# hpc-fci-mackenzie/cfrk

Measured on AMD Instinct MI355X. Metric: k-mers/sec, higher is better.
Workload: dtype u64; 1 GPU; 100000000 synthetic 150 bp reads, k=31, canonical, genome 100000000 (BASELINE.json configs[2]); reads=100000000, read_len=150, k=31, parallelism=read-shard x1

## Files before the change

### cfrk_amd/csrc/msp.hip

```cpp
#include "msp.h"
#include "table.h"
#include "msp_dev.h"

#include <algorithm>
#include <cmath>
#include <new>
#include <type_traits>
#include <vector>

namespace {
#include "msp_runs.h"

constexpr int P1_THREADS = 512;

constexpr int P2_THREADS = 512, P2_PER = 8;
constexpr int P2_GROUP = 4;

constexpr int P3_THREADS = 1024;
constexpr int TS_LOG = 12, TS = 1 << TS_LOG;

__device__ __noinline__ void spill_record(uint4 rec, int k, bool canon, TableView t, uint32_t weight = 1u) {
  t.stats[ST_SPILLED] = 1;
  dev_count_event(&t.stats[ST_AUX0]);
  const int nk = (int)(rec.w & 63u) + 1;
  const uint64_t hi = ((uint64_t)rec.x << 32) | rec.y;
  const uint64_t lo = (uint64_t)rec.z << 32;
  for (int j = 0; j < nk; ++j) {
    const uint64_t x = j ? ((hi << (2 * j)) | (lo >> (64 - 2 * j))) : hi;
    uint64_t key = x >> (64 - 2 * k);
    if (canon) {
      const uint64_t rc = dev_revcomp64(key, k);
      key = rc < key ? rc : key;
    }
    table_add1(t, key, weight);
  }
}

constexpr int P1_OWN = 61;
constexpr int P1_WAVES = P1_THREADS / 64;

__host__ __device__ __forceinline__ uint32_t l1_reg(uint32_t bin, uint32_t xg) { return xg * (uint32_t)B1 + bin; }
template <bool SUB>
__device__ __forceinline__ uint32_t bin_of(uint32_t w) { return SUB ? ((w >> 16) & (uint32_t)(B1 - 1)) : (w >> 16); }

template <bool EX>
__device__ __forceinline__ void l1_put(const MspView &v, uint32_t reg, uint32_t dst, uint4 rec, int k, bool canon,
                                       const TableView &t) {
  const bool exact1 = EX && v.exact1;
  const uint64_t cap = exact1 ? (uint64_t)v.rcap[reg] : v.cap1;
  const uint64_t at = exact1 ? v.rbase[reg] : (uint64_t)reg * v.cap1;
  if (dst < cap) {
    v.rec1[at + dst] = rec;
  } else if (exact1) {
    spill_record(rec, k, canon, t);
  } else if (*(volatile uint64_t *)&v.stats[ST_L1OVF] == 0) {
    const unsigned long long o = atomicAdd((unsigned long long *)&v.stats[ST_OVFN1], 1ull);
    if (o < v.ovf1_cap) v.ovf1[o] = rec;
    else v.stats[ST_L1OVF] = 1;
  }
}

constexpr int SUB_BITS = 5;
#define P1_MARK(text) asm volatile("; " text)
template <int P1B_TR, bool SUB = false>
struct P1Lds {
  static constexpr int STAGE = 4096 + 3 * 512 + P1B_TR * 128 + (SUB ? 2048 : 0);
  static constexpr int ARENA = P1_WAVES * STAGE;
  static constexpr int BYTES = ARENA + 2 * B1 * 4 + 32;
};

template <int W, int P1B_TR, bool EX, bool SUB>
__device__ __forceinline__ void p1_tile(uint4 *pool, const int8_t *__restrict__ data, int64_t nN, int k, int m, int canon,
                                        int64_t tile, uint32_t subreg, const MspView &v, const TableView &t) {
  constexpr int NH = 32 + W - 1;
  constexpr int P1B_STAGE = P1Lds<P1B_TR, SUB>::STAGE;
  constexpr int P1B_TAIL = B1 * 10;
  constexpr int P1B_RCAP = (P1_WAVES * P1B_STAGE - P1B_TAIL) / 16;
  uint4 *const arena = pool;
  uint32_t *const hist = reinterpret_cast<uint32_t *>(reinterpret_cast<uint8_t *>(pool) + P1Lds<P1B_TR, SUB>::ARENA);
  uint32_t *const loff = hist + B1;
  uint32_t *const wtot = loff + B1;
  uint32_t *const nrec_p = wtot + 4;
  uint32_t *const gbase = hist;
  unsigned long long *const dabs = reinterpret_cast<unsigned long long *>(reinterpret_cast<uint8_t *>(arena) + P1B_RCAP * 16);
  uint16_t *const plim = reinterpret_cast<uint16_t *>(dabs + B1);
  static_assert((P1_WAVES * P1B_STAGE - P1B_TAIL) % 16 == 0, "the table starts on a record boundary");

  const int nkmax = min(48 - k + 1, 32);
  const int tid = threadIdx.x, lane = tid & 63, wave = tid >> 6;
  uint8_t *const stage = reinterpret_cast<uint8_t *>(arena) + wave * P1B_STAGE;
  uint32_t *const s_str = reinterpret_cast<uint32_t *>(stage);
  uint4 *const s_EW = reinterpret_cast<uint4 *>(stage + 512);
  uint16_t *const s_leaf = reinterpret_cast<uint16_t *>(stage + 1536);
  uint16_t *const s_dsc = reinterpret_cast<uint16_t *>(stage + 4096 + 1536);
  uint8_t *const s_sub = stage + 4096 + 1536 + P1B_TR * 128;
  if (tid < B1) hist[tid] = 0;
  lds_barrier();

  P1_MARK("P1_PHASE_A");
  const int64_t wave_g = tile * P1_WAVES + wave;
  const int64_t chunk = wave_g * P1_OWN + lane - 1;
  const int64_t off = chunk * 32;
  uint32_t b0 = 0, b1 = 0, bad = 0xFFFFFFFFu;
  if (chunk >= 0) {
    if (off + 32 > nN) P1_MARK("P1_COLD byte-wise tail chunk");
    dev_load_chunk32(data, off, nN, b0, b1, bad);
  }
  const uint32_t n0 = dev_lane_next(b0), n1 = dev_lane_next(b1);
  const uint32_t nbad = dev_lane_next(bad), nnbad = dev_lane_next(dev_lane_next(bad));
  const uint64_t hi = ((uint64_t)b0 << 32) | b1;
  const uint64_t mid = ((uint64_t)n0 << 32) | n1;
  uint64_t Yh = ((uint64_t)bad << 32) | nbad, Yl = (uint64_t)nnbad << 32;
  {
    int w = 1;
#pragma unroll
    for (int st = 0; st < 5; ++st) {
      if (2 * w <= k) {
        Yh |= (Yh << w) | (Yl >> (64 - w));
        Yl |= Yl << w;
        w *= 2;
      }
    }
    if (k > w) {
      Yh |= (Yh << (k - w)) | (Yl >> (64 - (k - w)));
      Yl |= Yl << (k - w);
    }
  }
  const uint64_t Vx = ~Yh;
  const uint32_t V = (uint32_t)(Vx >> 32);
  const uint32_t prevV = dev_lane_prev(V) & 1u;

  uint32_t H[NH];
  const uint64_t Cx = msp_minimizers<W>(hi, mid, chunk, m, H);
  const uint64_t E = Cx | ~Vx | (1ull << (63 - NH));
  const uint32_t Vprev = (V >> 1) | (prevV << 31);
  uint32_t S = V & ((uint32_t)(Cx >> 32) | ~Vprev);
  const bool owner = lane >= 1 && lane <= P1_OWN && off < nN;
  if (!owner) S = 0;

  P1_MARK("P1_PHASE_B1");
  {
    const LeafPack LP = leaf_pack(H);
    uint4 *lp = reinterpret_cast<uint4 *>(s_leaf + lane * 32);
    lp[0] = make_uint4(LP.w[0], LP.w[1], LP.w[2], LP.w[3]);
    lp[1] = make_uint4(LP.w[4], LP.w[5], LP.w[6], LP.w[7]);
    lp[2] = make_uint4(LP.w[8], LP.w[9], LP.w[10], LP.w[11]);
    lp[3] = make_uint4(LP.w[12], LP.w[13], LP.w[14], LP.w[15]);
    reinterpret_cast<uint2 *>(s_str)[lane] = make_uint2(b0, b1);
    s_EW[lane] = make_uint4((uint32_t)E, (uint32_t)(E >> 32), ((uint32_t)Vx >> 1) | (V << 31), Vprev);
    if (SUB) {
      uint32_t sw[8];
#pragma unroll
      for (int i = 0; i < 8; ++i) {
        uint32_t x = 0;
#pragma unroll
        for (int j = 3; j >= 0; --j) {
          const uint32_t h = H[4 * i + j];
          x = (x << 8) | (((h >> 24) & 15u) << 1) | ((h >> 7) & 1u);
        }
        sw[i] = x;
      }
      uint4 *sp = reinterpret_cast<uint4 *>(s_sub + lane * 32);
      sp[0] = make_uint4(sw[0], sw[1], sw[2], sw[3]);
      sp[1] = make_uint4(sw[4], sw[5], sw[6], sw[7]);
    }
  }
  if (v.dbg & CFRK_ABL_P1_NO_EMIT) {
    if (S == 0x12345678u && (uint32_t)E == 0x9ABCDEFu) v.stats[ST_AUX0] = 1;
    return;
  }
  uint32_t cnt_w;
  uint32_t S2 = 0;
  const uint32_t wcap = (v.dbg & CFRK_DEBUG_SMALL_WAVE_CAP) ? 64u : (uint32_t)(P1B_TR * 64);
  {
    const uint32_t mine = (uint32_t)__popc(S);
    const uint32_t incl = dev_wave_scan_incl(mine);
    cnt_w = (uint32_t)__builtin_amdgcn_readlane((int)incl, 63);
    uint32_t widx = incl - mine;
    const uint32_t tag = (uint32_t)lane << 5;
    if (incl <= wcap) {
      uint16_t *dp = s_dsc + widx - 1;
      while (S) {
        const int a = __clz(S);
        S &= ~(0x80000000u >> a);
        *++dp = (uint16_t)(tag | (uint32_t)a);
      }
    } else {
      P1_MARK("P1_COLD wave over capacity");
      while (S) {
        const int a = __clz(S);
        const uint32_t bit = 0x80000000u >> a;
        S &= ~bit;
        if (widx < wcap) s_dsc[widx] = (uint16_t)(tag | (uint32_t)a);
        else S2 |= bit;
        ++widx;
      }
    }
  }
  lds_wave_sync();

  const uint32_t nkm1 = (uint32_t)(nkmax - 1);
  const int zc = 2 * (48 - k);
  auto build = [&](uint32_t d) {
    const uint4 ew = s_EW[d >> 5];
    const uint32_t leaf = s_leaf[d];
    const uint32_t idx0 = (d - 1u) >> 4, sh = 0u - 2u * d;
    const uint32_t D0 = s_str[idx0], D1 = s_str[idx0 + 1], D2 = s_str[idx0 + 2], D3 = s_str[idx0 + 3];
    const uint32_t a = d & 31u, na = ~d;
    const uint32_t e32 = __builtin_amdgcn_alignbit(ew.y, ew.x, na);
    const uint32_t nm1 = min((uint32_t)__clz(e32), nkm1);
    const uint32_t lf = (ew.w >> (na & 31u)) & 1u;
    const uint64_t Ws = ((uint64_t)ew.w << 32) | ew.z;
    const uint32_t rf = (uint32_t)((Ws << (a + nm1 + 2u)) >> 63);
    uint4 rec;
    rec.x = __builtin_amdgcn_alignbit(D0, D1, sh);
    const int z = zc - 2 * (int)nm1;
    uint64_t r12 = ((uint64_t)__builtin_amdgcn_alignbit(D1, D2, sh) << 32) | __builtin_amdgcn_alignbit(D2, D3, sh);
    r12 = (W < 8 && z >= 64) ? 0ull : (r12 & (~0ull << z));
    rec.y = (uint32_t)(r12 >> 32);
    rec.z = (uint32_t)r12;
    rec.w = (leaf << 8) | (rf << 7) | (lf << 6) | nm1;
    if (SUB) rec.w |= (uint32_t)s_sub[d] << 24;
    return rec;
  };

  while (S2) {
    P1_MARK("P1_COLD direct append");
    const int a = __clz(S2);
    S2 &= ~(0x80000000u >> a);
    const uint4 rec = build(((uint32_t)lane << 5) | (uint32_t)a);
    if (((rec.w >> 8) & v.sel_mask) != v.sel_val) continue;
    const uint32_t reg = l1_reg(bin_of<SUB>(rec.w), subreg);
    const uint32_t dst = atomicAdd(&v.cnt1[reg], 1u);
    l1_put<EX>(v, reg, dst, rec, k, canon != 0, t);
  }

  P1_MARK("P1_PHASE_B2");
  uint4 rc[P1B_TR];
  uint32_t rk[P1B_TR];
  cnt_w = min(cnt_w, wcap);
  auto emit = [&](auto sel) {
    if (decltype(sel)::value) P1_MARK("P1_COLD multi-pass selection");
#pragma unroll
    for (int tr = 0; tr < P1B_TR; ++tr) {
      rk[tr] = 0xFFFFFFFFu;
      const uint32_t i = (uint32_t)(tr * 64 + lane);
      if (i < cnt_w) {
        rc[tr] = build(s_dsc[i]);
        if (!decltype(sel)::value || ((rc[tr].w >> 8) & v.sel_mask) == v.sel_val)
          rk[tr] = atomicAdd(&hist[bin_of<SUB>(rc[tr].w)], 1u);
      }
    }
  };
  if (v.sel_mask == 0 && v.sel_val == 0) emit(std::false_type{});
  else emit(std::true_type{});
  lds_barrier();

  P1_MARK("P1_PHASE_C");
  uint32_t my_base = 0;
  if (tid < B1) {
    const uint32_t c = hist[tid];
    if (c) my_base = atomicAdd(&v.cnt1[l1_reg(tid, subreg)], c);
  }
  block_scan<B1, true>(hist, loff, wtot);
  if (tid == B1 - 1) *nrec_p = loff[tid] + hist[tid];
#pragma unroll
  for (int tr = 0; tr < P1B_TR; ++tr) {
    if (rk[tr] != 0xFFFFFFFFu) {
      const uint32_t pos = loff[bin_of<SUB>(rc[tr].w)] + rk[tr];
      if (pos < (uint32_t)P1B_RCAP) arena[pos] = rc[tr];
    }
  }
  if (tid < B1) {
    gbase[tid] = my_base;
    const uint32_t reg = l1_reg(tid, subreg);
    const bool exact1 = EX && v.exact1;
    const uint64_t cap = exact1 ? (uint64_t)v.rcap[reg] : v.cap1;
    const uint64_t at = exact1 ? v.rbase[reg] : (uint64_t)reg * v.cap1;
    const uint32_t lo = loff[tid];
    dabs[tid] = at + my_base - lo;
    const uint64_t room = cap > (uint64_t)my_base ? cap - my_base : 0;
    plim[tid] = (uint16_t)min((uint64_t)lo + room, (uint64_t)0xFFFFu);
    static_assert(P1B_RCAP <= 0xFFFF, "arena positions fit 16 bits");
  }
  lds_barrier();

  P1_MARK("P1_PHASE_D");
  const uint32_t nrec_s = *nrec_p;
  const uint32_t nrec = min(nrec_s, (uint32_t)P1B_RCAP);
  for (uint32_t p = tid; p < nrec; p += P1_THREADS) {
    const uint4 rec = arena[p];
    const uint32_t b = bin_of<SUB>(rec.w);
    if (p < (uint32_t)plim[b]) {
      v.rec1[dabs[b] + p] = rec;
    } else {
      P1_MARK("P1_COLD region full");
      l1_put<EX>(v, l1_reg(b, subreg), gbase[b] + (p - loff[b]), rec, k, canon != 0, t);
    }
  }
  if (nrec_s > (uint32_t)P1B_RCAP) {
    P1_MARK("P1_COLD arena overflow");
#pragma unroll
    for (int tr = 0; tr < P1B_TR; ++tr) {
      if (rk[tr] != 0xFFFFFFFFu) {
        const uint32_t b = bin_of<SUB>(rc[tr].w);
        if (loff[b] + rk[tr] >= (uint32_t)P1B_RCAP)
          l1_put<EX>(v, l1_reg(b, subreg), gbase[b] + rk[tr], rc[tr], k, canon != 0, t);
      }
    }
  }
}

template <int W, int P1B_TR, bool SUB>
__global__ __launch_bounds__(P1_THREADS, ((P1B_TR <= 6 && !SUB) ? 6 : 4)) void msp_p1b_kernel(const int8_t *__restrict__ data,
                                                             int64_t nN, int k, int m, int canon,
                                                             int64_t tile0, MspView v, TableView t) {
  __shared__ uint4 pool[P1Lds<P1B_TR, SUB>::BYTES / 16];
  const int64_t tile = tile0 + blockIdx.x;
  p1_tile<W, P1B_TR, true, SUB>(pool, data, nN, k, m, canon, tile, (uint32_t)tile & (v.nxg - 1), v, t);
}

constexpr int NCLS = 2;
constexpr int NSUB = NCLS * B2;
__device__ __forceinline__ uint32_t sub_of(uint32_t w) { return (((w >> 8) & (B2 - 1)) << 1) | ((((w >> 6) & 3u) == 3u) ? 1u : 0u); }

template <int PER>
struct P2Lds {
  static constexpr int TILE = P2_THREADS * PER;
  static constexpr int DABS = TILE * 16;
  static constexpr int HIST = DABS + NSUB * 8;
  static constexpr int LOFF = HIST + NSUB * 4;
  static constexpr int PLIM = LOFF + NSUB * 4;
  static constexpr int WTOT = PLIM + NSUB * 2;
  static constexpr int RPRE = WTOT + (P2_THREADS / 64) * 4;
  static constexpr int GPRE = RPRE + (NXG + 1) * 4;
  static constexpr int BYTES = (GPRE + (B1 / NXCD + 1) * 4 + 15) / 16 * 16;
};

template <int PER, bool EX, bool PF, int NGRP>
__device__ __forceinline__ void p2_item(uint4 *pool, uint32_t b1, uint32_t grp, int k, int canon, const MspView &v, const TableView &t) {
  constexpr int TILE = P2_THREADS * PER;
  static_assert(TILE <= 0xFFFF, "tile positions fit 16 bits");
  uint4 *const sorted = pool;
  uint8_t *const pb = reinterpret_cast<uint8_t *>(pool);
  unsigned long long *const dabs = reinterpret_cast<unsigned long long *>(pb + P2Lds<PER>::DABS);
  uint32_t *const hist = reinterpret_cast<uint32_t *>(pb + P2Lds<PER>::HIST);
  uint32_t *const loff = reinterpret_cast<uint32_t *>(pb + P2Lds<PER>::LOFF);
  uint16_t *const plim = reinterpret_cast<uint16_t *>(pb + P2Lds<PER>::PLIM);
  uint32_t *const wtot = reinterpret_cast<uint32_t *>(pb + P2Lds<PER>::WTOT);
  uint32_t *const rpre = reinterpret_cast<uint32_t *>(pb + P2Lds<PER>::RPRE);
  static_assert(NSUB <= P2_THREADS && NSUB % 64 == 0, "the scan below gives one thread per sub-bin");
  static_assert(NXG <= 64, "one wave scans the sub-region sizes");
  const int tid = threadIdx.x;
  const bool exact1 = EX && v.exact1, exact2 = EX && v.exact;
  if (tid < 64) {
    const uint32_t c = ((uint32_t)tid < v.nxg) ? (uint32_t)min((uint64_t)v.cnt1[l1_reg(b1, tid)],
                                                               exact1 ? (uint64_t)v.rcap[l1_reg(b1, tid)] : v.cap1) : 0u;
    const uint32_t incl = dev_wave_scan_incl(c);
    if ((uint32_t)tid < v.nxg) rpre[tid] = incl - c;
    if (tid == 63) rpre[v.nxg] = incl;
  }
  lds_barrier();
  const uint64_t n = rpre[v.nxg];
  const uint64_t g0r = (uint64_t)grp * NGRP * TILE;
  if (g0r >= n) return;
  uint32_t sr = 0;
  {
    uint32_t hi = v.nxg;
    const uint64_t idx = g0r + tid;
    while (hi - sr > 1) {
      const uint32_t mid = (sr + hi) >> 1;
      if (rpre[mid] <= idx) sr = mid; else hi = mid;
    }
  }
  auto fetch = [&](uint64_t idx) {
    while (sr + 1 < v.nxg && rpre[sr + 1] <= idx) ++sr;
    if (exact1) return v.rec1[v.rbase[l1_reg(b1, sr)] + (idx - rpre[sr])];
    return v.rec1[(uint64_t)l1_reg(b1, sr) * v.cap1 + (idx - rpre[sr])];
  };
  const uint4 zero4 = make_uint4(0u, 0u, 0u, 0u);
  uint4 nx[PF ? PER : 1];
  if (PF) {
#pragma unroll
    for (int i = 0; i < PER; ++i) {
      const uint64_t idx = g0r + (uint64_t)i * P2_THREADS + tid;
      nx[PF ? i : 0] = zero4;
      if (idx < n) nx[PF ? i : 0] = fetch(idx);
    }
  }
  for (int tt = 0; tt < NGRP; ++tt) {
    const uint64_t r0 = g0r + (uint64_t)tt * TILE;
    if (r0 >= n) break;
    const uint32_t nt = (uint32_t)min((uint64_t)TILE, n - r0);
    uint4 r[PER];
    if (PF) {
#pragma unroll
      for (int i = 0; i < PER; ++i) r[i] = nx[PF ? i : 0];
      if (tt + 1 < NGRP) {
#pragma unroll
        for (int i = 0; i < PER; ++i) {
          const uint64_t idx = r0 + TILE + (uint64_t)i * P2_THREADS + tid;
          nx[PF ? i : 0] = zero4;
          if (idx < n) nx[PF ? i : 0] = fetch(idx);
        }
      }
    } else {
#pragma unroll
      for (int i = 0; i < PER; ++i) {
        const uint64_t idx = r0 + (uint64_t)i * P2_THREADS + tid;
        r[i] = zero4;
        if (idx < n) r[i] = fetch(idx);
      }
    }
    if (tid < NSUB) hist[tid] = 0;
    lds_barrier();
#pragma unroll
    for (int i = 0; i < PER; ++i) {
      const uint32_t idx = (uint32_t)i * P2_THREADS + tid;
      if (idx < nt) atomicAdd(&hist[sub_of(r[i].w)], 1u);
    }
    lds_barrier();
    uint32_t g0 = 0;
    {
      const int lane = tid & 63, wave = tid >> 6;
      const bool mine = tid < NSUB;
      const uint32_t x0 = mine ? hist[tid] : 0u;
      if (x0 && !(v.dbg & CFRK_ABL_P2_NO_ATOMIC)) g0 = atomicAdd(&v.cnt2[b1 * NSUB + tid], x0);
      const uint32_t incl = dev_wave_scan_incl(x0);
      if (lane == 63) wtot[wave] = incl;
      lds_barrier();
      uint32_t bs = 0;
      for (int w = 0; w < wave; ++w) bs += wtot[w];
      if (mine) {
        loff[tid] = bs + incl - x0;
        hist[tid] = 0;
      }
      lds_barrier();
    }
#pragma unroll
    for (int i = 0; i < PER; ++i) {
      const uint32_t idx = (uint32_t)i * P2_THREADS + tid;
      if (idx < nt) {
        const uint32_t sb = sub_of(r[i].w);
        sorted[loff[sb] + atomicAdd(&hist[sb], 1u)] = r[i];
      }
    }
    if (tid < NSUB) {
      const uint64_t leaf = ((uint64_t)b1 * NSUB + tid) >> 1;
      const uint32_t cls = tid & 1u;
      uint64_t cap = cls ? v.cap2c : v.cap2t;
      uint64_t at = (leaf >> v.sel_bits) * (v.cap2c + v.cap2t) + (cls ? 0 : v.cap2c);
      if (exact2) { cap = v.lcap[b1 * NSUB + tid]; at = v.lbase[b1 * NSUB + tid]; }
      const uint32_t lo = loff[tid];
      dabs[tid] = at + g0 - lo;
      const uint64_t room = cap > (uint64_t)g0 ? cap - g0 : 0;
      plim[tid] = (uint16_t)min((uint64_t)lo + room, (uint64_t)0xFFFFu);
    }
    lds_barrier();
    for (uint32_t p = tid; p < nt; p += P2_THREADS) {
      const uint4 rec = sorted[p];
      const uint32_t sb = sub_of(rec.w);
      if (v.dbg & CFRK_ABL_P2_LINEAR_OUT) {
        v.rec2[(uint64_t)b1 * (NSUB / 2) * (v.cap2c + v.cap2t) + r0 + p] = rec;
        continue;
      }
      if (p < (uint32_t)plim[sb]) { v.rec2[dabs[sb] + p] = rec; continue; }
      const uint64_t leaf = ((uint64_t)b1 * NSUB + sb) >> 1;
      const uint32_t cls = sb & 1u;
      uint64_t cap = cls ? v.cap2c : v.cap2t;
      uint64_t at = (leaf >> v.sel_bits) * (v.cap2c + v.cap2t) + (cls ? 0 : v.cap2c);
      if (exact2) { cap = v.lcap[b1 * NSUB + sb]; at = v.lbase[b1 * NSUB + sb]; }
      const uint64_t dst = dabs[sb] + p - at;
      if (dst >= 0x80000000ull) v.stats[ST_CWRAP] = 1;
      if (dst < cap) v.rec2[at + dst] = rec;
      else if (exact2) spill_record(rec, k, canon != 0, t);
      else {
        if (*(volatile uint64_t *)&v.stats[ST_L2OVF] == 0) {
          const unsigned long long o = atomicAdd((unsigned long long *)&v.stats[ST_OVFN], 1ull);
          if (o < v.ovf_cap) v.ovf[o] = rec;
          else v.stats[ST_L2OVF] = 1;
        }
      }
    }
    lds_barrier();
  }
}

template <int PER, bool EX, bool PF>
__device__ __forceinline__ void p2_role(uint4 *pool, uint32_t wg, uint32_t nwg, int k, int canon, const MspView &v, const TableView &t) {
  constexpr int TILE = P2_THREADS * PER;
  uint32_t *const gpre = reinterpret_cast<uint32_t *>(reinterpret_cast<uint8_t *>(pool) + P2Lds<PER>::GPRE);
  constexpr int BPG = B1 / NXCD;
  static_assert(P2_THREADS == BPG * 16, "sixteen threads add up a bin's sub-regions");
  const int tid = threadIdx.x;
  const bool exact1 = EX && v.exact1;
  const uint32_t xg = wg & (NXCD - 1), j0 = wg / NXCD, nj = nwg / NXCD;
  {
    const uint32_t i = (uint32_t)tid >> 4, part = (uint32_t)tid & 15u, b = xg + NXCD * i;
    uint32_t sum = 0;
    for (uint32_t sr = part; sr < v.nxg; sr += 16u) {
      const uint32_t reg = l1_reg(b, sr);
      sum += (uint32_t)min((uint64_t)v.cnt1[reg], exact1 ? (uint64_t)v.rcap[reg] : v.cap1);
    }
#pragma unroll
    for (int d = 1; d < 16; d <<= 1) sum += __shfl_xor(sum, d);
    if (part == 0) gpre[i + 1] = (sum + (uint32_t)(TILE * P2_GROUP) - 1u) / (uint32_t)(TILE * P2_GROUP);
    if (tid == 0) gpre[0] = 0;
    lds_barrier();
    if (tid == 0) for (int q = 1; q <= BPG; ++q) gpre[q] += gpre[q - 1];
    lds_barrier();
  }
  const uint32_t nitems = gpre[BPG];
  uint32_t bi = 0;
  for (uint32_t item = j0; item < nitems; item += nj) {
    while (gpre[bi + 1] <= item) ++bi;
    p2_item<PER, EX, PF, P2_GROUP>(pool, xg + NXCD * bi, item - gpre[bi], k, canon, v, t);
  }
}

__global__ __launch_bounds__(P2_THREADS, 4) void msp_p2_kernel(int k, int canon, MspView v, TableView t) {
  __shared__ uint4 pool[(P2Lds<P2_PER>::BYTES + 15) / 16];
  p2_role<P2_PER, true, true>(pool, blockIdx.x, gridDim.x, k, canon, v, t);
}

__device__ __noinline__ void spill_kmer(TableView t, uint64_t key, uint32_t add) {
  if (key == CFRK_EMPTY_KEY) {
    atomicAdd((unsigned long long *)&t.stats[ST_ONES], (unsigned long long)add);
    return;
  }
  t.stats[ST_SPILLED] = 1;
  dev_count_event(&t.stats[ST_AUX1]);
  table_add1(t, key, add);
}

constexpr int NBUCKET = TS / 2;
__device__ __forceinline__ uint32_t lds_bucket(uint64_t key) {
  return (((uint32_t)key ^ (uint32_t)(key >> 32)) * 0x9E3779B1u) >> (32 - (TS_LOG - 1));
}

constexpr int KT_TRIPS = 64;
constexpr int KT_TRIPS_SPLIT = 16;

constexpr uint32_t KT_DONE = 0x80000000u;
template <bool SAT = false>
__device__ __forceinline__ void kt_try(unsigned long long *keys, uint32_t *cnts, uint64_t key, uint32_t &b,
                                       uint32_t add) {
  const bool p = (int32_t)b >= 0;
  const uint32_t bb = b & (NBUCKET - 1);
  const ulonglong2 q = reinterpret_cast<const ulonglong2 *>(keys)[bb];
  const bool m0 = q.x == key, m1 = q.y == key;
  const bool e0 = q.x == CFRK_EMPTY_KEY, e1 = q.y == CFRK_EMPTY_KEY;
  const bool hit = m0 || m1;
  const uint32_t s = 2 * bb + ((m0 || (!m1 && e0)) ? 0u : 1u);
  uint32_t won = 0u;
  if (p && !hit && (e0 || e1)) {
    const unsigned long long old = atomicCAS(&keys[s], (unsigned long long)CFRK_EMPTY_KEY, (unsigned long long)key);
    won = (old == CFRK_EMPTY_KEY || old == key) ? 1u : 0u;
  }
  const bool ok = hit || won != 0u;
  if (SAT) {
    if (p && ok) {
      const uint32_t old = atomicAdd(&cnts[s], add);
      if (old > CFRK_COUNT_MAX - add) atomicExch(&cnts[s], CFRK_COUNT_MAX);
    }
  } else atomicAdd(&cnts[s], (p && ok) ? add : 0u);
  const bool full = !(hit || e0 || e1);
  const uint32_t nb = full ? ((bb + 1) & (NBUCKET - 1)) : bb;
  b = (p && !ok) ? nb : (b | KT_DONE);
}

__device__ __forceinline__ void kt_count(unsigned long long *keys, uint32_t *cnts, uint64_t key, uint32_t add,
                                         bool valid, const TableView &t) {
  uint32_t b = lds_bucket(key) | (valid ? 0u : KT_DONE);
  add = min(add, CFRK_COUNT_MAX);
  for (int it = 0; it < KT_TRIPS && __ballot((int32_t)b >= 0); ++it) kt_try<true>(keys, cnts, key, b, add);
  if ((int32_t)b >= 0) spill_kmer(t, key, add);
}

struct KeySubset { uint32_t mask, val; };
__device__ __forceinline__ bool in_subset(uint64_t key, KeySubset ss) {
  return (((((uint32_t)key ^ (uint32_t)(key >> 32)) * 0x9E3779B1u) >> 8) & ss.mask) == ss.val;
}

template <bool CANON>
__device__ __forceinline__ void count_record_v2(unsigned long long *keys, uint32_t *cnts, uint4 rec, uint32_t add,
                                                bool valid, int k, uint64_t kmask, int rcsh,
                                                const TableView &t, KeySubset ss = KeySubset{0u, 0u},
                                                uint32_t *ovf = nullptr, int part = 0, int parts = 1,
                                                const uint8_t *tb = nullptr, uint32_t tb_n = 0u) {
  if (ovf && *(volatile uint32_t *)ovf) return;
  const int nall = valid ? (int)(rec.w & 63u) + 1 : 0;
  const int per = (parts == 1) ? nall : (parts == 2) ? ((nall + 1) >> 1) : ((nall + 2) / 3);
  const int j0 = part * per;
  const int nk = max(min(nall, j0 + per) - j0, 0);
  uint64_t hi = ((uint64_t)rec.x << 32) | rec.y;
  uint64_t lo = (uint64_t)rec.z << 32;
  if (parts != 1 && j0) {
// ... 2052 lines not shown
```

### cfrk_amd/csrc/msp_dev.h

```cpp
#pragma once
#include "common.h"

constexpr int B1_LOG = 8, B2_LOG = 8;
constexpr int B1 = 1 << B1_LOG, B2 = 1 << B2_LOG;
constexpr int NXCD = 8;
constexpr int NXG = 64;
constexpr int NLEAF = B1 * B2;


__device__ __forceinline__ uint32_t hash_mmer(uint32_t c) { return c * 0x9E3779B1u; }
__device__ __forceinline__ uint32_t leaf_of(uint32_t wmin) { return (wmin >> 8) & 0xFFFFu; }

struct LeafPack { uint32_t w[16]; };
template <int N>
__device__ __forceinline__ LeafPack leaf_pack(const uint32_t (&H)[N]) {
  LeafPack L;
#pragma unroll
  for (int i = 0; i < 16; ++i)
    L.w[i] = __builtin_amdgcn_perm(H[2 * i + 1], H[2 * i], 0x06050201u);
  return L;
}
__device__ __forceinline__ uint32_t leaf_pick(const LeafPack &L, int a) {
  const bool c16 = (a & 16) != 0, c8 = (a & 8) != 0, c4 = (a & 4) != 0, c2 = (a & 2) != 0;
#define CFRK_SEL(c, hi_, lo_) ({ const uint32_t x_ = (lo_), y_ = (hi_); (c) ? y_ : x_; })
  const uint32_t s0 = CFRK_SEL(c16, L.w[8], L.w[0]), s1 = CFRK_SEL(c16, L.w[9], L.w[1]);
  const uint32_t s2 = CFRK_SEL(c16, L.w[10], L.w[2]), s3 = CFRK_SEL(c16, L.w[11], L.w[3]);
  const uint32_t s4 = CFRK_SEL(c16, L.w[12], L.w[4]), s5 = CFRK_SEL(c16, L.w[13], L.w[5]);
  const uint32_t s6 = CFRK_SEL(c16, L.w[14], L.w[6]), s7 = CFRK_SEL(c16, L.w[15], L.w[7]);
  const uint32_t e0 = CFRK_SEL(c8, s4, s0), e1 = CFRK_SEL(c8, s5, s1), e2 = CFRK_SEL(c8, s6, s2);
  const uint32_t e3 = CFRK_SEL(c8, s7, s3);
  const uint32_t f0 = CFRK_SEL(c4, e2, e0), f1 = CFRK_SEL(c4, e3, e1);
  const uint32_t g = CFRK_SEL(c2, f1, f0);
#undef CFRK_SEL
  return (g >> ((a & 1) << 4)) & 0xFFFFu;
}

__device__ __forceinline__ void lds_barrier() { asm volatile("s_waitcnt lgkmcnt(0)\n\ts_barrier" ::: "memory"); }
__device__ __forceinline__ void lds_wave_sync() {
  asm volatile("s_waitcnt lgkmcnt(0)" ::: "memory");
  __builtin_amdgcn_wave_barrier();
}

template <int NW>
__device__ __forceinline__ void wave_append(uint32_t (&set)[NW], const uint32_t (&mine)[NW], bool keep, unsigned long long mask, int c, int n) {
  const int lane = threadIdx.x & 63;
  const int rank = (int)__builtin_amdgcn_mbcnt_hi((uint32_t)(mask >> 32), __builtin_amdgcn_mbcnt_lo((uint32_t)mask, 0u));
  const int dst = keep ? (c + rank) : ((c + n) & 63);
  const int da = dst << 2;
  const bool take = lane >= c && lane < c + n;
#pragma unroll
  for (int i = 0; i < NW; ++i) {
    const uint32_t p = __builtin_amdgcn_ds_permute(da, mine[i]);
    set[i] = take ? p : set[i];
  }
}

__device__ __forceinline__ unsigned long long noted_counts8(const uint8_t *tb, uint32_t tb_n, int j0) {
  unsigned long long hist = 0ull;
  for (uint32_t e = 0; __ballot(e < tb_n); ++e) {
    if (e < tb_n) {
      const int d = min(max((int)tb[e] - j0, 0), 8);
      hist += 1ull << (7 * d);
    }
  }
  unsigned long long exq = 0ull;
  uint32_t run = 0;
#pragma unroll
  for (int d = 8; d >= 1; --d) {
    run += (uint32_t)(hist >> (7 * d)) & 127u;
    exq |= (unsigned long long)run << (8 * (d - 1));
  }
  return exq;
}

template <int NIT, int NT, class Occ>
__device__ __forceinline__ void wg_rank_slots(uint32_t (&wbase)[NIT], uint32_t *wg_total, Occ occupied) {
  const int tid = threadIdx.x, lane = tid & 63;
#pragma unroll
  for (int i = 0; i < NIT; ++i) {
    const unsigned long long m = __ballot(occupied(i * NT + tid));
    uint32_t b = 0;
    if (lane == 0 && m) b = atomicAdd(wg_total, (uint32_t)__popcll(m));
    wbase[i] = __shfl(b, 0);
  }
}
template <int NIT, int NT, class Occ, class Emit>
__device__ __forceinline__ void wg_emit_slots(const uint32_t (&wbase)[NIT], unsigned long long list_base, Occ occupied, Emit emit) {
  const int tid = threadIdx.x, lane = tid & 63;
#pragma unroll
  for (int i = 0; i < NIT; ++i) {
    const int s = i * NT + tid;
    const bool occ = occupied(s);
    const unsigned long long m = __ballot(occ);
    if (occ) emit(s, list_base + wbase[i] + __popcll(m & ((1ull << lane) - 1ull)));
  }
}

template <int NB, bool LDS_ONLY = false>
__device__ __forceinline__ void block_scan(const uint32_t *cnt, uint32_t *off, uint32_t *wtot) {
  const int tid = threadIdx.x, lane = tid & 63, wave = tid >> 6;
  uint32_t x = 0, incl = 0;
  if (tid < NB) {
    x = cnt[tid];
    incl = dev_wave_scan_incl(x);
    if (lane == 63) wtot[wave] = incl;
  }
  if (LDS_ONLY) lds_barrier(); else __syncthreads();
  if (tid < NB) {
    uint32_t base = 0;
    for (int w = 0; w < wave; ++w) base += wtot[w];
    off[tid] = base + incl - x;
  }
  if (LDS_ONLY) lds_barrier(); else __syncthreads();
}

template <int W>
__device__ __forceinline__ uint64_t msp_minimizers(uint64_t hi, uint64_t mid, int64_t chunk, int m,
                                                   uint32_t (&H)[32 + W - 1]) {
  constexpr int NH = 32 + W - 1;
  constexpr int P = (W >= 16) ? 16 : (W >= 8) ? 8 : (W >= 4) ? 4 : 2;
  static_assert(W < 32, "position tags are 5 bits");
  {
    (void)chunk;
    const uint32_t D[3] = {(uint32_t)(hi >> 32), (uint32_t)hi, (uint32_t)(mid >> 32)};
    uint32_t R[4];
#pragma unroll
    for (int i = 0; i < 3; ++i) {
      uint32_t x = __brev(D[i]);
      x = ((x >> 1) & 0x55555555u) | ((x & 0x55555555u) << 1);
      R[3 - i] = ~x;
    }
    R[0] = 0;
    const uint32_t mmask = (m == 16) ? 0xFFFFFFFFu : ((1u << (2 * m)) - 1u);
    const int fsh = 32 - 2 * m;
#pragma unroll
    for (int j = 0; j < 32; ++j) {
      const int o = 2 * j, q = o >> 5, r = o & 31;
      const uint32_t X = r ? __builtin_amdgcn_alignbit(D[q], D[q + 1], 32 - r) : D[q];
      const int o2 = 96 - 2 * j, q2 = o2 >> 5, r2 = o2 & 31;
      const uint32_t Y = r2 ? __builtin_amdgcn_alignbit(R[q2], R[q2 + 1], 32 - r2) : R[q2];
      const uint32_t fm = X >> fsh, rm = Y & mmask;
      H[j] = (hash_mmer(min(fm, rm)) & ~127u) | (uint32_t)j;
    }
  }
#pragma unroll
  for (int j = 0; j < W - 1; ++j) H[32 + j] = dev_lane_next(H[j]);
  if (W >= 8) {
    uint32_t Pm[32];
#pragma unroll
    for (int i = 1; i < 32; ++i) {
      const int q = i + W - 1;
      Pm[i] = (q % W == 0) ? H[q] : min(Pm[(q % W == 0) ? i : i - 1], H[q]);
    }
    constexpr int LASTB = (31 / W) * W + W - 1;
#pragma unroll
    for (int j = (LASTB < NH ? LASTB : NH - 1) - 1; j >= 0; --j)
      if ((j + 1) % W != 0) H[j] = min(H[j], H[j + 1]);
#pragma unroll
    for (int i = 1; i < 32; ++i) H[i] = min(H[i], Pm[i]);
  } else {
#pragma unroll
    for (int s = 1; s < P; s <<= 1) {
#pragma unroll
      for (int j = 0; j + s < NH; ++j) H[j] = min(H[j], H[j + s]);
    }
    if (W > P) {
#pragma unroll
      for (int i = 0; i < 32; ++i) H[i] = min(H[i], H[i + W - P]);
    }
  }
  auto push = [](uint32_t &acc, uint32_t a, uint32_t b) {
    asm("v_cmp_ne_u32_e32 vcc, %1, %2\n\tv_addc_co_u32_e32 %0, vcc, %0, %0, vcc" : "+v"(acc) : "v"(a), "v"(b) : "vcc");
  };
  const uint32_t prevW = dev_lane_prev(H[31]);
  uint32_t ch = 0;
  push(ch, H[0], prevW);
#pragma unroll
  for (int p = 1; p < 32; ++p) push(ch, H[p], H[p - 1]);
  const uint32_t cl = dev_lane_next(ch) & ~(0xFFFFFFFFu >> (W - 1));
  return ((uint64_t)ch << 32) | cl;
}
```

Baseline: 444.2 billion k-mers/s.

## Fast-path validity smear, fuse halo min via DPP, pack per-bin output table

Adds a wave-uniform fast path for the k-mer validity smear when each lane has at most one bad bit, replacing the log-step shift loop with an arithmetic smear. It trims the minimizer halo exchange to only the lanes needed and fuses the cross-lane move with the min using a DPP v_min instruction. It also replaces the separate dabs/plim LDS tables with one 16-byte otab entry per bin, comparing 64-bit destinations directly. These reduce ALU and cross-lane work in phase 1, but the extra LDS tail shrinks arena capacity slightly, and the inline DPP asm relies on exact wave-shift semantics.

```diff
diff --git a/cfrk_amd/csrc/msp.hip b/cfrk_amd/csrc/msp.hip
--- a/cfrk_amd/csrc/msp.hip
+++ b/cfrk_amd/csrc/msp.hip
@@ -74,7 +74,7 @@
                                         int64_t tile, uint32_t subreg, const MspView &v, const TableView &t) {
   constexpr int NH = 32 + W - 1;
   constexpr int P1B_STAGE = P1Lds<P1B_TR, SUB>::STAGE;
-  constexpr int P1B_TAIL = B1 * 10;
+  constexpr int P1B_TAIL = B1 * 16;
   constexpr int P1B_RCAP = (P1_WAVES * P1B_STAGE - P1B_TAIL) / 16;
   uint4 *const arena = pool;
   uint32_t *const hist = reinterpret_cast<uint32_t *>(reinterpret_cast<uint8_t *>(pool) + P1Lds<P1B_TR, SUB>::ARENA);
@@ -82,8 +82,7 @@
   uint32_t *const wtot = loff + B1;
   uint32_t *const nrec_p = wtot + 4;
   uint32_t *const gbase = hist;
-  unsigned long long *const dabs = reinterpret_cast<unsigned long long *>(reinterpret_cast<uint8_t *>(arena) + P1B_RCAP * 16);
-  uint16_t *const plim = reinterpret_cast<uint16_t *>(dabs + B1);
+  ulonglong2 *const otab = reinterpret_cast<ulonglong2 *>(arena + P1B_RCAP);
   static_assert((P1_WAVES * P1B_STAGE - P1B_TAIL) % 16 == 0, "the table starts on a record boundary");
 
   const int nkmax = min(48 - k + 1, 32);
@@ -98,6 +97,7 @@
   lds_barrier();
 
   P1_MARK("P1_PHASE_A");
+  P1_MARK("P1_SUB_LOAD");
   const int64_t wave_g = tile * P1_WAVES + wave;
   const int64_t chunk = wave_g * P1_OWN + lane - 1;
   const int64_t off = chunk * 32;
@@ -107,11 +107,20 @@
     dev_load_chunk32(data, off, nN, b0, b1, bad);
   }
   const uint32_t n0 = dev_lane_next(b0), n1 = dev_lane_next(b1);
-  const uint32_t nbad = dev_lane_next(bad), nnbad = dev_lane_next(dev_lane_next(bad));
   const uint64_t hi = ((uint64_t)b0 << 32) | b1;
   const uint64_t mid = ((uint64_t)n0 << 32) | n1;
-  uint64_t Yh = ((uint64_t)bad << 32) | nbad, Yl = (uint64_t)nnbad << 32;
-  {
+  P1_MARK("P1_SUB_CORE");
+  uint64_t Yh;
+  if (__ballot((bad & (bad - 1u)) != 0u) == 0ull) {
+    const uint32_t t = bad << (k - 1);
+    const uint32_t carry = __builtin_elementwise_sub_sat(bad >> (32 - k), 1u);
+    const uint32_t yh = (t - bad) | t | dev_lane_next(carry);
+    Yh = ((uint64_t)yh << 32) | dev_lane_next(yh);
+  } else {
+    P1_MARK("P1_COLD general validity smear");
+    const uint32_t nbad = dev_lane_next(bad), nnbad = dev_lane_next(dev_lane_next(bad));
+    uint64_t Yl = (uint64_t)nnbad << 32;
+    Yh = ((uint64_t)bad << 32) | nbad;
     int w = 1;
 #pragma unroll
     for (int st = 0; st < 5; ++st) {
@@ -257,6 +266,7 @@
   lds_barrier();
 
   P1_MARK("P1_PHASE_C");
+  P1_MARK("P1_SUB_RESERVE");
   uint32_t my_base = 0;
   if (tid < B1) {
     const uint32_t c = hist[tid];
@@ -264,6 +274,7 @@
   }
   block_scan<B1, true>(hist, loff, wtot);
   if (tid == B1 - 1) *nrec_p = loff[tid] + hist[tid];
+  P1_MARK("P1_SUB_ARENA");
 #pragma unroll
   for (int tr = 0; tr < P1B_TR; ++tr) {
     if (rk[tr] != 0xFFFFFFFFu) {
@@ -271,6 +282,7 @@
       if (pos < (uint32_t)P1B_RCAP) arena[pos] = rc[tr];
     }
   }
+  P1_MARK("P1_SUB_TABLE");
   if (tid < B1) {
     gbase[tid] = my_base;
     const uint32_t reg = l1_reg(tid, subreg);
@@ -278,10 +290,7 @@
     const uint64_t cap = exact1 ? (uint64_t)v.rcap[reg] : v.cap1;
     const uint64_t at = exact1 ? v.rbase[reg] : (uint64_t)reg * v.cap1;
     const uint32_t lo = loff[tid];
-    dabs[tid] = at + my_base - lo;
-    const uint64_t room = cap > (uint64_t)my_base ? cap - my_base : 0;
-    plim[tid] = (uint16_t)min((uint64_t)lo + room, (uint64_t)0xFFFFu);
-    static_assert(P1B_RCAP <= 0xFFFF, "arena positions fit 16 bits");
+    otab[tid] = make_ulonglong2(at + my_base - lo, at + max(cap, (uint64_t)my_base));
   }
   lds_barrier();
 
@@ -291,8 +300,10 @@
   for (uint32_t p = tid; p < nrec; p += P1_THREADS) {
     const uint4 rec = arena[p];
     const uint32_t b = bin_of<SUB>(rec.w);
-    if (p < (uint32_t)plim[b]) {
-      v.rec1[dabs[b] + p] = rec;
+    const ulonglong2 ot = otab[b];
+    const uint64_t dst = ot.x + p;
+    if (dst < ot.y) {
+      v.rec1[dst] = rec;
     } else {
       P1_MARK("P1_COLD region full");
       l1_put<EX>(v, l1_reg(b, subreg), gbase[b] + (p - loff[b]), rec, k, canon != 0, t);
diff --git a/cfrk_amd/csrc/msp_dev.h b/cfrk_amd/csrc/msp_dev.h
--- a/cfrk_amd/csrc/msp_dev.h
+++ b/cfrk_amd/csrc/msp_dev.h
@@ -114,6 +114,12 @@
   if (LDS_ONLY) lds_barrier(); else __syncthreads();
 }
 
+__device__ __forceinline__ uint32_t dev_min_lane_next(uint32_t a, uint32_t b) {
+  uint32_t d;
+  asm("s_nop 1\n\tv_min_u32_dpp %0, %1, %2 wave_shl:1 row_mask:0xf bank_mask:0xf bound_ctrl:1" : "=v"(d) : "v"(b), "v"(a));
+  return d;
+}
+
 template <int W>
 __device__ __forceinline__ uint64_t msp_minimizers(uint64_t hi, uint64_t mid, int64_t chunk, int m,
                                                    uint32_t (&H)[32 + W - 1]) {
@@ -143,18 +149,22 @@
       H[j] = (hash_mmer(min(fm, rm)) & ~127u) | (uint32_t)j;
     }
   }
+  constexpr int LASTB = (31 / W) * W + W - 1;
+  constexpr int SEND = LASTB < NH ? LASTB : NH - 1;
+  constexpr int NHALO = (W >= 8) ? SEND - 31 : W - 1;
 #pragma unroll
-  for (int j = 0; j < W - 1; ++j) H[32 + j] = dev_lane_next(H[j]);
+  for (int j = 0; j < NHALO; ++j) H[32 + j] = dev_lane_next(H[j]);
   if (W >= 8) {
     uint32_t Pm[32];
 #pragma unroll
     for (int i = 1; i < 32; ++i) {
       const int q = i + W - 1;
-      Pm[i] = (q % W == 0) ? H[q] : min(Pm[(q % W == 0) ? i : i - 1], H[q]);
+      if (q < 32 + NHALO) Pm[i] = (q % W == 0) ? H[q] : min(Pm[(q % W == 0) ? i : i - 1], H[q]);
+      else if (q % W == 0) Pm[i] = dev_lane_next(H[q - 32]);
+      else Pm[i] = dev_min_lane_next(Pm[i - 1], H[q - 32]);
     }
-    constexpr int LASTB = (31 / W) * W + W - 1;
 #pragma unroll
-    for (int j = (LASTB < NH ? LASTB : NH - 1) - 1; j >= 0; --j)
+    for (int j = SEND - 1; j >= 0; --j)
       if ((j + 1) % W != 0) H[j] = min(H[j], H[j + 1]);
 #pragma unroll
     for (int i = 1; i < 32; ++i) H[i] = min(H[i], Pm[i]);
```

Measured after the change: 447.1 billion k-mers/s, median of 6. No clear change (+0.7%).
